# SamArgt/AudioSourceSep

Measured on AMD Instinct MI355X. Metric: Glow fwd+logdet passes/sec on 64×64×1 mel tiles (K=32,L=3), 1→8 MI355X, higher is better.
Workload: dtype f16x3

## Files before the change

### audiosourcesep_amd/csrc/glowk_co.h

```cpp
#pragma once
#include "glowk_kernels.h"

constexpr int CO_PX = 128;
constexpr int CO_PSTR = 132;

template <int KIN, int MOUT, int NF, int MODE>
struct RingC {
  static constexpr int MODE7 = net_dir<MODE>;
  using S = RingS<KIN, MOUT, NF, MODE7, 2>;
  static constexpr bool FUSE = (MODE & NET_FUSE) != 0;
  static constexpr bool SAVE = MODE7 == NET_FWD_SAVE, BWD = MODE7 == NET_BWD;
  static constexpr bool MERGE = S::NMT <= 3;
  static constexpr bool M0LAST = S::NMT % 3 == 2;
  static constexpr bool STORE = (MODE & NET_STORE) != 0;
  static constexpr int MODEX = net_dir<MODE> | (MODE & NET_STORE);
  static constexpr int NFH = S::NFH, NRB = S::NRB, NMT = S::NMT, KS = S::KS;
  static constexpr int UNITP = S::MAINP / 2;
  static constexpr int UNIT4 = S::MAIN4 / 2;
  static constexpr int PPW = UNITP / 4;
  static constexpr int NG = NFH / 2;
  static constexpr int K1PW = (S::K1P + 3) / 4;
  static constexpr int EPN = BWD ? 0 : S::EPN;
  static constexpr int MASKN = BWD ? 2 * 4 * NF * 64 : 0;
  static constexpr size_t LDS_BYTES = (size_t)3 * UNIT4 * 16 + (size_t)2 * S::K14 * 16 + (size_t)EPN * 4 + (size_t)MASKN * 2 +
                                      (FUSE ? (size_t)36 * CO_PSTR * 4 + CO_PX * 16 : 0);
  static constexpr bool FITS = (MODE7 == NET_FWD || MODE7 == NET_FWD2 || SAVE || BWD) && !(MODE & NET_HALF) && (!STORE || ((SAVE || BWD) && !FUSE)) && S::NGRP == 1 && (NMT == 2 || NMT == 3 || (NMT == 5 && !STORE && !BWD)) &&
                               (!FUSE || (MOUT == 36 && !BWD)) && KS <= 3 && NF % 4 == 0 && NFH >= 2 && NFH % 2 == 0 && UNITP % 4 == 0 && PPW == NG &&
                               2 * LDS_BYTES <= 160 * 1024 + 1;
  static constexpr int XST = STORE ? 8 : 0;
  static constexpr int z_acts(int z) { int n = 0; for (int t = z * NFH; t < (z + 1) * NFH; ++t) n += (t % NMT == 0) ? 1 : 0; return n; }
  static constexpr int z_st(int z) { return STORE ? z_acts(z) * (8 + (SAVE ? 1 : 0)) : 0; }
  __device__ static const float4* main_unit(const float4* img, int pass, int i, int half) { return S::main_chunk(img, pass, i) + (size_t)half * UNIT4; }
  __device__ static const float4* out_unit(const float4* img, int pass, int z) { return S::out_chunk(img, pass, 0) + (size_t)z * UNIT4; }
};

__device__ __forceinline__ void co_bar() {
  __builtin_amdgcn_s_waitcnt(0xC07F);
  h3_barrier();
}

template <int N>
__device__ __forceinline__ void co_end() {
  __builtin_amdgcn_s_waitcnt((N & 15) | 0x0070 | ((N >> 4) << 14));
  h3_barrier();
}
template <int N>
__device__ __forceinline__ void co_end_st(bool more) {
  if (more) co_end<N + 1>();
  else co_end<N>();
}
// ... 38 lines not shown
    acc2[o1][1] = __builtin_amdgcn_mfma_f32_16x16x32_f16(af[3], bh[1], acc2[o1][1], 0, 0, 0);
    if (MODE7 != NET_FWD2) {
      acc2[o0][0] = __builtin_amdgcn_mfma_f32_16x16x32_f16(af[0], bl[0], acc2[o0][0], 0, 0, 0);
      acc2[o0][1] = __builtin_amdgcn_mfma_f32_16x16x32_f16(af[0], bl[1], acc2[o0][1], 0, 0, 0);
      acc2[o1][0] = __builtin_amdgcn_mfma_f32_16x16x32_f16(af[2], bl[0], acc2[o1][0], 0, 0, 0);
      acc2[o1][1] = __builtin_amdgcn_mfma_f32_16x16x32_f16(af[2], bl[1], acc2[o1][1], 0, 0, 0);
    }
    acc2[o0][0] = __builtin_amdgcn_mfma_f32_16x16x32_f16(af[0], bh[0], acc2[o0][0], 0, 0, 0);
    acc2[o0][1] = __builtin_amdgcn_mfma_f32_16x16x32_f16(af[0], bh[1], acc2[o0][1], 0, 0, 0);
    acc2[o1][0] = __builtin_amdgcn_mfma_f32_16x16x32_f16(af[2], bh[0], acc2[o1][0], 0, 0, 0);
    acc2[o1][1] = __builtin_amdgcn_mfma_f32_16x16x32_f16(af[2], bh[1], acc2[o1][1], 0, 0, 0);
    __builtin_amdgcn_sched_barrier(0);
  }
}

template <int KIN, int MOUT, int NF, int MODE, int PASS, bool SOLO, int Z>
__device__ __forceinline__ void co_Z(const NetArgs& a, const H3Ctx& hc, const CoCtx& c, const float* epl, float* pl,
                                     f32x4 (&acc2)[(RingC<KIN, MOUT, NF, MODE>::NRB)][2], f32x4 (&acc3)[(RingC<KIN, MOUT, NF, MODE>::NMT)][2], h8 (&bh)[2],
                                     h8 (&bl)[2], const int (&q)[2], const bool (&qok)[2], int lane, int kq,
                                     f32x4 (&keep)[(RingC<KIN, MOUT, NF, MODE>::NMT)][2]) {
  using G = RingC<KIN, MOUT, NF, MODE>;
  constexpr int NFH = G::NFH, NMT = G::NMT, M3 = MOUT, MODE7 = G::MODE7;
  constexpr bool NEXT = !SOLO && PASS == 0;
  constexpr bool LAST = !SOLO && PASS == 1;
  if constexpr (NMT == 3) {
    if constexpr (Z == 0) stage4<G::UNITP, 70>(G::out_unit(c.img, PASS, 2), c.m1, c.w4, c.voff);
    if constexpr (Z == 1 && NEXT) stage4<G::UNITP, 71>(G::out_unit(c.img, PASS + 1, 0), c.d, c.w4, c.voff);
    if constexpr (Z == 2 && NEXT) stage4<G::UNITP, 72>(G::main_unit(c.img, PASS + 1, 0, 0), c.m0, c.w4, c.voff);
  } else if constexpr (NMT == 2) {
    if constexpr (Z == 0 && NEXT) stage4<G::UNITP, 75>(G::main_unit(c.img, PASS + 1, 0, 1), c.m1, c.w4, c.voff);
    if constexpr (Z == 1 && NEXT) stage4<G::UNITP, 76>(G::out_unit(c.img, PASS + 1, 0), c.d, c.w4, c.voff);
  } else {
    static_assert(NMT == 5, "conv3 units");
    if constexpr (Z == 0) stage4<G::UNITP, 80>(G::out_unit(c.img, PASS, 2), c.m1, c.w4, c.voff);
    if constexpr (Z == 1) stage4<G::UNITP, 81>(G::out_unit(c.img, PASS, 3), c.d, c.w4, c.voff);
    if constexpr (Z == 2) stage4<G::UNITP, 82>(G::out_unit(c.img, PASS, 4), c.m0, c.w4, c.voff);
    if constexpr (Z == 3 && NEXT) stage4<G::UNITP, 83>(G::main_unit(c.img, PASS + 1, 0, 1), c.m1, c.w4, c.voff);
    if constexpr (Z == 4 && NEXT) stage4<G::UNITP, 84>(G::out_unit(c.img, PASS + 1, 0), c.d, c.w4, c.voff);
  }
  const float4* slot = Z % 3 == 0 ? c.d : Z % 3 == 1 ? c.m0 : c.m1;
  const h8* buf = reinterpret_cast<const h8*>(slot) + lane;
  const float* pb = epl + NF * 32;
#pragma unroll
  for (int tp = 0; tp < NFH; ++tp) {
    const int t = Z * NFH + tp;
    const int fo = t / NMT, ml = t % NMT;
    if (ml == 0) {
      unsigned mask = 0, bits = 0;
      if (G::BWD) mask = hc.mkl[((size_t)(threadIdx.x >> 6) * NF + PASS * NFH + fo) * 64 + lane];
      if constexpr (G::STORE)
        bits = h3s_act_pair<MODE7, true>(acc2[2 * fo][0], acc2[2 * fo + 1][0], acc2[2 * fo][1], acc2[2 * fo + 1][1], a.sc2, mask, bh, bl,
                                         uniform_fptr(a.st2 + (size_t)(PASS * NFH + fo) * 32 * a.Q), ((unsigned)(4 * kq) * (unsigned)a.Q + (unsigned)q[0]) * 4u,
                                         (unsigned)a.Q * 4u);
// ... 16 lines not shown
#pragma unroll
        for (int r = 0; r < 4; ++r) {
          const int m = ml * 16 + 4 * kq + r;
          const float part = G::BWD ? acc3[ml][hf][r] * (a.sc3 * hc.ub[hf]) : PASS == 0 ? fmaf(acc3[ml][hf][r], a.sc3, pb[m]) : acc3[ml][hf][r] * a.sc3;
          if constexpr (NEXT && G::MERGE) { keep[ml][hf][r] = part; continue; }
          const float val = (LAST && G::MERGE) ? part + keep[ml][hf][r] : part;
          if constexpr (G::FUSE) {
            if (m < M3) pl[m * CO_PSTR + (int)(threadIdx.x >> 6) * 32 + 16 * hf + (lane & 15)] = val;
          } else {
            float* Pp = a.P + ((SOLO || !G::MERGE) ? (size_t)PASS * a.pstride : (size_t)0);
            if (m < M3 && qok[hf]) Pp[(size_t)m * a.Q + q[hf]] = val;
          }
        }
    }
  }
  constexpr bool ISSUED = NMT == 3 ? (Z == 0 || NEXT) : NMT == 2 ? (Z <= 1 && NEXT) : (Z <= 2 || NEXT);
  if constexpr (Z + 1 < NMT) {
    if constexpr (G::STORE) {
      constexpr int after = (ISSUED ? G::PPW : 0) + G::z_st(Z) + ((NMT == 3 && Z == 1) ? G::z_st(0) : 0);
      co_end<(after < 63 ? after : 63)>();
    } else if constexpr (G::SAVE) co_end<0>();
    else co_end<(ISSUED ? G::PPW : 0)>();
  } else co_bar();
}

template <int KIN, int MOUT, int NF, int MODE, int PASS, bool SOLO>
__device__ __forceinline__ void co_pass(const NetArgs& a, const H3Ctx& hc, const CoCtx& c, const float* epl, float* pl,
                                        const h8 (&xh)[(RingC<KIN, MOUT, NF, MODE>::KS)][2], const h8 (&xl)[(RingC<KIN, MOUT, NF, MODE>::KS)][2],
                                        const int (&q)[2], const bool (&qok)[2], int lane, int kq, f32x4 (&keep)[(RingC<KIN, MOUT, NF, MODE>::NMT)][2]) {
  using G = RingC<KIN, MOUT, NF, MODE>;
  using S = typename G::S;
  constexpr int NRB = G::NRB, NFH = G::NFH, MODE7 = G::MODE7;
  constexpr int f2base = PASS * NFH * 32;
  constexpr bool SECOND = !SOLO && PASS == 1;
  f32x4 acc2[NRB][2];
#pragma unroll
  for (int ob = 0; ob < NRB; ++ob)
#pragma unroll
    for (int r = 0; r < 4; ++r) {
      const float b = G::BWD ? 0.0f : epl[f2base + ob * 16 + 4 * kq + r];
      acc2[ob][0][r] = b;
      acc2[ob][1][r] = b;
    }
  const bool st = G::SAVE && PASS == 0 && hc.wok;
  constexpr int XST = PASS == 0 ? G::XST : 0;
  h8 bh[2], bl[2];
#pragma nounroll
  for (int i0 = 0; i0 < NF; i0 += 2) {
    if (i0 > 0 || (SECOND && !G::M0LAST)) stage4<G::UNITP, 73>(G::main_unit(c.img, PASS, i0, 1), c.m1, c.w4, c.voff);
// ... 5 lines not shown
    else co_end_st<G::PPW + XST>(st);
    co_Y<NFH, MODE7, 0, 1, S::K1P>(c.m0, bh, bl, acc2, lane, hc.k1img + (size_t)((i0 + 2) % NF) * S::K14, hc.k1s0, c.w4, c.voff);
    co_end_st<G::K1PW + XST>(st);
    co_Y<NFH, MODE7, 1, 2, S::K1P>(c.m1, bh, bl, acc2, lane, G::main_unit(c.img, PASS, i0 + 1, 0), c.m0, c.w4, c.voff);
    co_bar();
    stage4<G::UNITP, 74>(G::main_unit(c.img, PASS, i0 + 1, 1), c.m1, c.w4, c.voff);
    h3s_X<KIN, MOUT, NF, G::MODEX, 2, 1, PASS, G::STORE>(a, hc, i0 + 1, xh, xl, lane, bh, bl);
    co_end_st<G::PPW + XST>(st);
    co_Y<NFH, MODE7, 0, 3, S::K1P>(c.m0, bh, bl, acc2, lane, hc.k1img + (size_t)((i0 + 3) % NF) * S::K14, hc.k1s1, c.w4, c.voff);
    co_end_st<G::K1PW + XST>(st);
    co_Y<NFH, MODE7, 1, 4, S::K1P>(c.m1, bh, bl, acc2, lane, i0 + 2 < NF ? G::main_unit(c.img, PASS, i0 + 2, 0) : G::out_unit(c.img, PASS, 1), c.m0,
                                   c.w4, c.voff);
    co_bar();
  }
  f32x4 acc3[G::NMT][2];
  co_Z<KIN, MOUT, NF, MODE, PASS, SOLO, 0>(a, hc, c, epl, pl, acc2, acc3, bh, bl, q, qok, lane, kq, keep);
  co_Z<KIN, MOUT, NF, MODE, PASS, SOLO, 1>(a, hc, c, epl, pl, acc2, acc3, bh, bl, q, qok, lane, kq, keep);
  if constexpr (G::NMT >= 3) co_Z<KIN, MOUT, NF, MODE, PASS, SOLO, 2>(a, hc, c, epl, pl, acc2, acc3, bh, bl, q, qok, lane, kq, keep);
  if constexpr (G::NMT >= 4) co_Z<KIN, MOUT, NF, MODE, PASS, SOLO, 3>(a, hc, c, epl, pl, acc2, acc3, bh, bl, q, qok, lane, kq, keep);
  if constexpr (G::NMT >= 5) co_Z<KIN, MOUT, NF, MODE, PASS, SOLO, 4>(a, hc, c, epl, pl, acc2, acc3, bh, bl, q, qok, lane, kq, keep);
}

template <int KIN, int MOUT, int NF, int MODE, bool SPLIT>
__global__ __launch_bounds__(256, 2) void k_net_h3c(NetArgs a) {
  using G = RingC<KIN, MOUT, NF, MODE>;
  using S = typename G::S;
  constexpr int KS = G::KS;
  constexpr int SGN = G::BWD ? -1 : 1;
  static_assert(G::FITS, "shape");
  static_assert(!(G::FUSE && SPLIT), "the fused coupling needs both passes in one workgroup");

  const int tid = threadIdx.x;
  __shared__ __attribute__((aligned(1024))) float4 slotM0[G::UNIT4];
  __shared__ __attribute__((aligned(1024))) float4 slotM1[G::UNIT4];
  __shared__ __attribute__((aligned(1024))) float4 slotD[G::UNIT4];
  __shared__ __attribute__((aligned(1024))) float4 k1slot0[S::K14];
  __shared__ __attribute__((aligned(1024))) float4 k1slot1[S::K14];
  float* epl = nullptr;
  if constexpr (!G::BWD) { __shared__ float epl_arr[S::EPN]; epl = epl_arr; }
  unsigned short* mkl = nullptr;
  if constexpr (G::BWD) { __shared__ __attribute__((aligned(1024))) unsigned short mkl_arr[G::MASKN]; mkl = mkl_arr; }
  float* plds = nullptr;
  float4* vstash = nullptr;
  if constexpr (G::FUSE) {
    __shared__ float plds_arr[36 * CO_PSTR];
// ... 6 lines not shown
  const int kq = lane >> 4;
  const int qbase = ((int)blockIdx.x * 4 + wave) * 32;
  const int q[2] = {G::STORE ? qbase + 2 * n16 : qbase + n16, G::STORE ? qbase + 2 * n16 + 1 : qbase + 16 + n16};
  const bool qok[2] = {q[0] < a.Q, q[1] < a.Q};
  const int pass0 = SPLIT ? (int)blockIdx.y : 0;

  H3Ctx hc;
  hc.sA = hc.sB = hc.sD = nullptr; hc.k1s0 = k1slot0; hc.k1s1 = k1slot1;
  hc.k1img = a.RSp; hc.img = a.RSp; hc.mkl = mkl; hc.mk2off = 4 * NF * 64; hc.pl = plds;
  hc.wblk = (size_t)blockIdx.x * 4 + wave;
  hc.wok = (long)hc.wblk * 32 < a.Q;
  hc.w4 = wave; hc.voff = (unsigned)lane * 16u; hc.ub[0] = hc.ub[1] = 1.0f;
  CoCtx c;
  c.m0 = slotM0; c.m1 = slotM1; c.d = slotD; c.img = a.RSp; c.w4 = wave; c.voff = (unsigned)lane * 16u;

  stage4<G::UNITP, 60>(G::main_unit(c.img, pass0, 0, 0), slotM0, c.w4, c.voff);
  stage4<G::UNITP, 61>(G::main_unit(c.img, pass0, 0, 1), slotM1, c.w4, c.voff);
  stage4<G::UNITP, 62>(G::out_unit(c.img, pass0, 0), slotD, c.w4, c.voff);
  stage4<S::K1P, 63>(hc.k1img, k1slot0, c.w4, c.voff);
  stage4<S::K1P, 64>(hc.k1img + S::K14, k1slot1, c.w4, c.voff);
  if constexpr (G::BWD) {
    stage4<NF / 2, 65>(reinterpret_cast<const float4*>(a.mask1 + (size_t)blockIdx.x * 4 * NF * 64), reinterpret_cast<float4*>(mkl), c.w4, c.voff);
    stage4<NF / 2, 66>(reinterpret_cast<const float4*>(a.mask2 + (size_t)blockIdx.x * 4 * NF * 64), reinterpret_cast<float4*>(mkl + 4 * NF * 64), c.w4, c.voff);
  }

  h8 xh[KS][2], xl[KS][2];
  float xmax = 0.0f;
  {
    const int hw = a.h * a.w;
#pragma unroll
    for (int hf = 0; hf < 2; ++hf) {
      const int qq = qok[hf] ? q[hf] : 0;
      const int rem = qq % hw;
      const int i = rem / a.w, j0 = rem % a.w;
      const float* base = a.vin + (long)qq * a.in_stride + a.in_off;
      if constexpr (G::BWD) {
        float v[KS][8];
        float pm = 0.0f;
#pragma unroll
        for (int s = 0; s < KS; ++s) {
          gather8<KIN, false, SGN>(base, i, j0, a.h, a.w, a.in_stride, qok[hf], 32 * s + 8 * kq, v[s]);
          pm = range8(pm, v[s]);
        }
        pm = nan_max(pm, __shfl_xor(pm, 16, 64));
        pm = nan_max(pm, __shfl_xor(pm, 32, 64));
        xmax = nan_max(xmax, pm);
        const float fac = G::STORE ? 1.0f : pixel_norm(pm, a.bnorm, hc.ub[hf]);
#pragma unroll
        for (int s = 0; s < KS; ++s) {
#pragma unroll
          for (int j = 0; j < 8; ++j) v[s][j] *= fac;
          split8(v[s], xh[s][hf], xl[s][hf]);
        }
      } else if constexpr (S::STK) {
        xmax = gather_stacked<KIN, SGN, G::MODE7 == NET_FWD2, KS, S::KSX>(base, i, j0, a.h, a.w, a.in_stride, qok[hf], kq, xh, xl, hf, xmax);
      } else {
#pragma unroll
        for (int s = 0; s < KS; ++s) {
          float v[8];
          gather8<KIN, true, SGN>(base, i, j0, a.h, a.w, a.in_stride, qok[hf], 32 * s + 8 * kq, v);
          xmax = range8(xmax, v);
          split8(v, xh[s][hf], xl[s][hf]);
        }
      }
    }
  }
  if constexpr (G::FUSE) {
    if (tid < CO_PX) {
      const int qv = (int)blockIdx.x * CO_PX + tid;
      vstash[tid] = qv < a.Q ? *reinterpret_cast<const float4*>(a.vin + (size_t)qv * 4) : float4{0.f, 0.f, 0.f, 0.f};
    }
  }
  if constexpr (!G::BWD)
    for (int i = tid; i < S::EPN; i += 256) epl[i] = a.eph[i];
  if (((G::BWD && !G::STORE) ? !(xmax <= 3.0e38f) : !(xmax <= a.xlim)) && a.flag) *a.flag = 1;
  if (a.xmax_out) range_probe(a.xmax_out, xmax);
  asm volatile("s_waitcnt vmcnt(0)" ::: "memory");
  __syncthreads();

  f32x4 keep[G::NMT][2];
  if constexpr (SPLIT) {
    if (pass0 == 0) co_pass<KIN, MOUT, NF, MODE, 0, true>(a, hc, c, epl, plds, xh, xl, q, qok, lane, kq, keep);
    else co_pass<KIN, MOUT, NF, MODE, 1, true>(a, hc, c, epl, plds, xh, xl, q, qok, lane, kq, keep);
  } else {
    co_pass<KIN, MOUT, NF, MODE, 0, false>(a, hc, c, epl, plds, xh, xl, q, qok, lane, kq, keep);
    co_pass<KIN, MOUT, NF, MODE, 1, false>(a, hc, c, epl, plds, xh, xl, q, qok, lane, kq, keep);
  }
  if constexpr (G::FUSE) {
    __syncthreads();
    fused_couple<CO_PX, CO_PSTR>(a, plds, vstash, tid);
  }
}
```

### audiosourcesep_amd/csrc/glowk_kernels.h

```cpp
#pragma once
#include "glowk_act_scale.h"

#include <hip/hip_runtime.h>
#include <utility>
#include <stdint.h>

typedef float f32x16 __attribute__((ext_vector_type(16)));

#define GLOWK_GPTR(p) ((const __attribute__((address_space(1))) void*)(p))
#define GLOWK_LPTR(p) ((__attribute__((address_space(3))) void*)(p))

__device__ __forceinline__ int mfma_row(int r, int hh) { return (r & 3) + 8 * (r >> 2) + 4 * hh; }

struct NetArgs {
  const float* vin;
  int in_stride, in_off;
  int Q, h, w;
  const float* K1p;
  const float* ep;
  const float4* R0p;
  unsigned short* mask1;
  unsigned short* mask2;
  float* P;
  size_t pstride;
// ... 1225 lines not shown
  f32x4 acc3[G::G0N][2];
  h3s_tail<KIN, MOUT, NF, MODE, NP, P0, PASS, SOLO>(a, c, epl, acc2, acc3, bh, bl, g, q, qok, lane, kq, keep, std::make_integer_sequence<int, 2 * G::NCH>());
}

template <int KIN, int MOUT, int NF, int MODE, int NP, int PASS, int P0>
__device__ __forceinline__ void h3s_passes(const NetArgs& a, const H3Ctx& c, const float* epl, const h8 (&xh)[(RingS<KIN, MOUT, NF, MODE, NP>::KS)][2],
                                           const h8 (&xl)[(RingS<KIN, MOUT, NF, MODE, NP>::KS)][2], int g, const int (&q)[2], const bool (&qok)[2], int lane, int kq,
                                           f32x4 (&keep)[(RingS<KIN, MOUT, NF, MODE, NP>::G0N)][2]) {
  h3s_pass<KIN, MOUT, NF, MODE, NP, P0, PASS, false>(a, c, epl, xh, xl, g, q, qok, lane, kq, keep);
  if constexpr (PASS + 1 < NP) h3s_passes<KIN, MOUT, NF, MODE, NP, PASS + 1, (RingS<KIN, MOUT, NF, MODE, NP>::NCH + 1 + P0) & 1>(a, c, epl, xh, xl, g, q, qok, lane, kq, keep);
}

__device__ __forceinline__ bool fz_not_finite(float v) { return !(fabsf(v) <= 3.0e38f); }

template <int PXW = 256, int PSTR = FUSE_PSTR>
__device__ __forceinline__ void fused_couple(const NetArgs& a, const float* pl, const float4* vst, int tid) {
  const int wave = tid >> 6, lane = tid & 63;
  const int px = wave * 32 + (lane & 31), k = lane >> 5;
  const int q = (int)blockIdx.x * PXW + px;
  const bool qok = q < a.Q;
  const int w = a.w, hw = a.h * a.w, nrows = PXW / w;
  const int pp = (qok ? q : 0) % hw;
  const int i = pp / w, j = pp % w, r = px / w;
  float ols = 0.0f, ot = 0.0f;
  bool missing = false;
#pragma unroll
  for (int tap = 0; tap < 9; ++tap) {
    const int dy = tap / 3 - 1, dx = tap % 3 - 1;
    const int ii = i + dy, jj = j + dx;
    if (ii < 0 || ii >= a.h || jj < 0 || jj >= w) continue;
    const int rr = r + dy;
    if (rr < 0 || rr >= nrows) { missing = true; continue; }
    const int spx = px + dy * w + dx;
    ols += pl[(tap * 4 + k) * PSTR + spx];
// ... 15 lines not shown
    bool bad = fz_not_finite(ols) | fz_not_finite(ot) | fz_not_finite(yk);
    if (bad && a.flag) *a.flag = 1;
    float z0, z1;
    if (a.fz_A) {
      z0 = a.fz_b[2 * k]; z1 = a.fz_b[2 * k + 1];
#pragma unroll
      for (int ci = 0; ci < 4; ++ci) {
        z0 = fmaf(y[ci], a.fz_A[ci * 4 + 2 * k], z0);
        z1 = fmaf(y[ci], a.fz_A[ci * 4 + 2 * k + 1], z1);
      }
    } else {
      z0 = y[2 * k]; z1 = y[2 * k + 1];
    }
    *reinterpret_cast<float2*>(a.fz_out + (size_t)q * a.fz_out_stride + a.fz_out_off + 2 * k) = float2{z0, z1};
  } else if (qok) {
    float* e = a.fz_edge + (((size_t)blockIdx.x * 4 + (r == 0 ? 0 : 1)) * FUSE_EW + j) * 4;
    e[k] = ols;
    e[2 + k] = ot;
  }
  for (int te = tid; te < 2 * w * 4; te += 2 * PXW) {
    const int which = te / (4 * w), jt = (te / 4) % w, ch = te & 3;
    float hsum = 0.0f;
#pragma unroll
    for (int dx = -1; dx <= 1; ++dx) {
      const int js = jt + dx;
      if (js < 0 || js >= w) continue;
      const int tap = (which ? 0 : 6) + dx + 1;
      hsum += pl[(tap * 4 + ch) * PSTR + (which ? (nrows - 1) * w : 0) + js];
    }
    a.fz_edge[(((size_t)blockIdx.x * 4 + 2 + which) * FUSE_EW + jt) * 4 + ch] = hsum;
  }
  if (a.fz_ldpart) {
    double d = (double)lsum;
#pragma unroll
    for (int o = 32; o > 0; o >>= 1) d += __shfl_down(d, o, 64);
    if (lane == 0) a.fz_ldpart[(size_t)blockIdx.x * (PXW / 32) + wave] = d;
  }
}

template <int KIN, int MOUT, int NF, int MODE, int NP, bool SPLIT>
__global__ __launch_bounds__(512, 2) void k_net_h3s(NetArgs a) {
  using G = RingS<KIN, MOUT, NF, MODE, NP>;
  constexpr int KS = G::KS;
  constexpr int SGN = (net_dir<MODE> == NET_BWD) ? -1 : 1;
  static_assert(G::FITS, "shape");

  __shared__ float4 slotA[G::MAIN4];
  __shared__ float4 slotB[G::MAIN4];
  __shared__ float4 slotD[G::MAIN4];
  __shared__ float4 k1slot0[G::K14];
  __shared__ float4 k1slot1[G::K14];
// ... 97 lines not shown
  f32x4 keep[G::G0N][2];
  if (g) h3_barrier();
  if constexpr (SPLIT) {
    if (solo_pass == 0) h3s_pass<KIN, MOUT, NF, MODE, NP, 0, 0, true>(a, c, epl, xh, xl, g, q, qok, lane, kq, keep);
    else if (solo_pass == 1) h3s_pass<KIN, MOUT, NF, MODE, NP, 0, 1, true>(a, c, epl, xh, xl, g, q, qok, lane, kq, keep);
    else if constexpr (NP > 2) {
      if (solo_pass == 2) h3s_pass<KIN, MOUT, NF, MODE, NP, 0, 2, true>(a, c, epl, xh, xl, g, q, qok, lane, kq, keep);
      else h3s_pass<KIN, MOUT, NF, MODE, NP, 0, 3, true>(a, c, epl, xh, xl, g, q, qok, lane, kq, keep);
    }
  } else {
    h3s_passes<KIN, MOUT, NF, MODE, NP, 0, 0>(a, c, epl, xh, xl, g, q, qok, lane, kq, keep);
  }
  if (!g) h3_barrier();
  if constexpr (G::FUSE) {
    __syncthreads();
    fused_couple(a, plds, vstash, tid);
  }
}
```

### audiosourcesep_amd/csrc/glowk_launch.h

```cpp
#pragma once
#include "glowk_kernels.h"
#include "glowk_co.h"
#include "glowk_q.h"

#include <cstdlib>
#include <string>

#define GLOWK_NET_SHAPES(X) X(2, 16) X(4, 16) X(8, 16) X(16, 16) X(2, 12) X(4, 12) X(8, 12) X(16, 12) \
                            X(2, 8) X(4, 8) X(8, 8) X(16, 8) X(2, 4) X(4, 4) X(8, 4) X(16, 4)

enum NetArith { NET_EXACT, NET_SPLIT3, NET_SPLIT2 };
struct NetCall { int dir; NetArith arith; bool store = false; };

enum NetFamily { FAM_F32, FAM_H3, FAM_H3S, FAM_H3S_HALF, FAM_FUSED, FAM_CO, FAM_Q, FAM_COUNT };

struct NetLaunch {
  int np = 0;
  int family = FAM_F32;
  bool co = false;
  bool q = false;
  int fused_px = 0;
  bool failed = false;
  explicit operator bool() const { return np > 0 || fused_px > 0; }
};
// ... 53 lines not shown
  return {};
}

template <class Kernel>
inline bool co_two_per_cu(Kernel kernel) {
  static int blocks = -1;
  if (blocks < 0) {
    int n = 0;
    if (hipOccupancyMaxActiveBlocksPerMultiprocessor(&n, kernel, 256, 0) != hipSuccess) { (void)hipGetLastError(); n = 0; }
    blocks = n;
  }
  return blocks >= 2;
}

template <int KIN, int MOUT, int NF, int MODE>
NetLaunch launch_h3s(const NetArgs& a, hipStream_t s, bool dry) {
  static_assert(!(MODE & NET_STORE), "no storing launches here: the co-resident branch does not check Q % 128 (launch_co_train does)");
  constexpr bool F2 = RingS<KIN, MOUT, NF, MODE, 2>::FITS, F4 = RingS<KIN, MOUT, NF, MODE, 4>::FITS;
  const int wgs = (a.Q + 255) / 256, cus = num_cus();
  if constexpr (F4) {
    if (a.max_np >= 4 && (4 * wgs <= cus || !F2)) {
      const bool split = 4 * wgs <= cus;
      if (!dry) {
        if (split) hipLaunchKernelGGL((k_net_h3s<KIN, MOUT, NF, MODE, 4, true>), dim3(wgs, 4), dim3(512), 0, s, a);
        else hipLaunchKernelGGL((k_net_h3s<KIN, MOUT, NF, MODE, 4, false>), dim3(wgs), dim3(512), 0, s, a);
      }
      return {4, FAM_H3S};
    }
  }
  if constexpr (F2) {
    const bool split = 2 * wgs <= cus;
    if constexpr (RingC<KIN, MOUT, NF, MODE>::FITS) {
      const int wgc = (a.Q + CO_PX - 1) / CO_PX;
      const bool co_ok = a.co && !env().co_off;
      if (co_ok && wgc > cus) {
        if constexpr (RingC<KIN, MOUT, NF, MODE | NET_FUSE>::FITS) {
          if (a.fuse && co_two_per_cu(k_net_h3c<KIN, MOUT, NF, MODE | NET_FUSE, false>)) {
            if (!dry) hipLaunchKernelGGL((k_net_h3c<KIN, MOUT, NF, MODE | NET_FUSE, false>), dim3(wgc), dim3(256), 0, s, a);
            return {0, FAM_FUSED, true, false, CO_PX};
          }
        }
        if (!a.fuse && co_two_per_cu(k_net_h3c<KIN, MOUT, NF, MODE, false>)) {
          if (!dry) hipLaunchKernelGGL((k_net_h3c<KIN, MOUT, NF, MODE, false>), dim3(wgc), dim3(256), 0, s, a);
          return {RingC<KIN, MOUT, NF, MODE>::MERGE ? 1 : 2, FAM_H3S, true};
        }
      }
      if (co_ok && split && wgc <= cus && a.max_np >= 2 && co_two_per_cu(k_net_h3c<KIN, MOUT, NF, MODE, true>)) {
        if (!dry) hipLaunchKernelGGL((k_net_h3c<KIN, MOUT, NF, MODE, true>), dim3(wgc, 2), dim3(256), 0, s, a);
        return {2, FAM_H3S, true};
      }
    }
    if constexpr ((MODE == NET_FWD || MODE == NET_FWD2 || MODE == NET_FWD_SAVE) && MOUT == 36) {
      if constexpr (RingS<KIN, MOUT, NF, MODE | NET_FUSE, 2>::FITS && RingS<KIN, MOUT, NF, MODE | NET_FUSE, 2>::MERGE) {
        if (a.fuse && !split) {
          if (!dry) hipLaunchKernelGGL((k_net_h3s<KIN, MOUT, NF, MODE | NET_FUSE, 2, false>), dim3(wgs), dim3(512), 0, s, a);
          return {0, FAM_FUSED, false, false, 256};
        }
      }
// ... 170 lines not shown
```

Before: 15960.

## Make co-resident forward net kernel persistent with cross-block weight and input prefetch

Forward co-resident net kernels with stacked input now run as persistent workgroups. The grid is capped at two per CU and each workgroup loops over pixel blocks. During the second pass the next block's first weight units are prefetched into LDS, and the next block's input gather is issued before the fused coupling epilogue, so the prologue of each new block overlaps the tail of the previous one. This is meant to hide per-workgroup startup costs: staging weights, gathering inputs, loading epilogue parameters, and launching many waves. In exchange it adds loop control, more registers to hold in-flight inputs, and conditional wait counts, and it threads an explicit block index through fused_couple.

```diff
diff --git a/audiosourcesep_amd/csrc/glowk_co.h b/audiosourcesep_amd/csrc/glowk_co.h
--- a/audiosourcesep_amd/csrc/glowk_co.h
+++ b/audiosourcesep_amd/csrc/glowk_co.h
@@ -34,6 +34,9 @@
   __device__ static const float4* out_unit(const float4* img, int pass, int z) { return S::out_chunk(img, pass, 0) + (size_t)z * UNIT4; }
 };
 
+template <int KIN, int MOUT, int NF, int MODE, bool SPLIT>
+constexpr bool co_persistent = !SPLIT && (net_dir<MODE> == NET_FWD || net_dir<MODE> == NET_FWD2) && !(MODE & NET_STORE) && RingC<KIN, MOUT, NF, MODE>::S::STK;
+
 __device__ __forceinline__ void co_bar() {
   __builtin_amdgcn_s_waitcnt(0xC07F);
   h3_barrier();
@@ -102,29 +105,33 @@
   }
 }
 
-template <int KIN, int MOUT, int NF, int MODE, int PASS, bool SOLO, int Z>
+template <int KIN, int MOUT, int NF, int MODE, int PASS, bool SOLO, int Z, bool PERS = false>
 __device__ __forceinline__ void co_Z(const NetArgs& a, const H3Ctx& hc, const CoCtx& c, const float* epl, float* pl,
                                      f32x4 (&acc2)[(RingC<KIN, MOUT, NF, MODE>::NRB)][2], f32x4 (&acc3)[(RingC<KIN, MOUT, NF, MODE>::NMT)][2], h8 (&bh)[2],
                                      h8 (&bl)[2], const int (&q)[2], const bool (&qok)[2], int lane, int kq,
-                                     f32x4 (&keep)[(RingC<KIN, MOUT, NF, MODE>::NMT)][2]) {
+                                     f32x4 (&keep)[(RingC<KIN, MOUT, NF, MODE>::NMT)][2], bool more = false) {
   using G = RingC<KIN, MOUT, NF, MODE>;
   constexpr int NFH = G::NFH, NMT = G::NMT, M3 = MOUT, MODE7 = G::MODE7;
+  constexpr bool NEXTB = PERS && !SOLO && PASS == 1;
   constexpr bool NEXT = !SOLO && PASS == 0;
+  constexpr bool NEXTD = NEXT || NEXTB;
   constexpr bool LAST = !SOLO && PASS == 1;
+  constexpr int NPASS = NEXTB ? 0 : PASS + 1;
+  const bool nx = !NEXTB || more;
   if constexpr (NMT == 3) {
     if constexpr (Z == 0) stage4<G::UNITP, 70>(G::out_unit(c.img, PASS, 2), c.m1, c.w4, c.voff);
-    if constexpr (Z == 1 && NEXT) stage4<G::UNITP, 71>(G::out_unit(c.img, PASS + 1, 0), c.d, c.w4, c.voff);
-    if constexpr (Z == 2 && NEXT) stage4<G::UNITP, 72>(G::main_unit(c.img, PASS + 1, 0, 0), c.m0, c.w4, c.voff);
+    if constexpr (Z == 1 && NEXTD) { if (nx) stage4<G::UNITP, 71>(G::out_unit(c.img, NPASS, 0), c.d, c.w4, c.voff); }
+    if constexpr (Z == 2 && NEXTD) { if (nx) stage4<G::UNITP, 72>(G::main_unit(c.img, NPASS, 0, 0), c.m0, c.w4, c.voff); }
   } else if constexpr (NMT == 2) {
-    if constexpr (Z == 0 && NEXT) stage4<G::UNITP, 75>(G::main_unit(c.img, PASS + 1, 0, 1), c.m1, c.w4, c.voff);
-    if constexpr (Z == 1 && NEXT) stage4<G::UNITP, 76>(G::out_unit(c.img, PASS + 1, 0), c.d, c.w4, c.voff);
+    if constexpr (Z == 0 && NEXTD) { if (nx) stage4<G::UNITP, 75>(G::main_unit(c.img, NPASS, 0, 1), c.m1, c.w4, c.voff); }
+    if constexpr (Z == 1 && NEXTD) { if (nx) stage4<G::UNITP, 76>(G::out_unit(c.img, NPASS, 0), c.d, c.w4, c.voff); }
   } else {
     static_assert(NMT == 5, "conv3 units");
     if constexpr (Z == 0) stage4<G::UNITP, 80>(G::out_unit(c.img, PASS, 2), c.m1, c.w4, c.voff);
     if constexpr (Z == 1) stage4<G::UNITP, 81>(G::out_unit(c.img, PASS, 3), c.d, c.w4, c.voff);
     if constexpr (Z == 2) stage4<G::UNITP, 82>(G::out_unit(c.img, PASS, 4), c.m0, c.w4, c.voff);
-    if constexpr (Z == 3 && NEXT) stage4<G::UNITP, 83>(G::main_unit(c.img, PASS + 1, 0, 1), c.m1, c.w4, c.voff);
-    if constexpr (Z == 4 && NEXT) stage4<G::UNITP, 84>(G::out_unit(c.img, PASS + 1, 0), c.d, c.w4, c.voff);
+    if constexpr (Z == 3 && NEXTD) { if (nx) stage4<G::UNITP, 83>(G::main_unit(c.img, NPASS, 0, 1), c.m1, c.w4, c.voff); }
+    if constexpr (Z == 4 && NEXTD) { if (nx) stage4<G::UNITP, 84>(G::out_unit(c.img, NPASS, 0), c.d, c.w4, c.voff); }
   }
   const float4* slot = Z % 3 == 0 ? c.d : Z % 3 == 1 ? c.m0 : c.m1;
   const h8* buf = reinterpret_cast<const h8*>(slot) + lane;
@@ -171,25 +178,29 @@
         }
     }
   }
-  constexpr bool ISSUED = NMT == 3 ? (Z == 0 || NEXT) : NMT == 2 ? (Z <= 1 && NEXT) : (Z <= 2 || NEXT);
+  constexpr bool ISSUED = NMT == 3 ? (Z == 0 || NEXTD) : NMT == 2 ? (Z <= 1 && NEXTD) : (Z <= 2 || NEXTD);
   if constexpr (Z + 1 < NMT) {
     if constexpr (G::STORE) {
       constexpr int after = (ISSUED ? G::PPW : 0) + G::z_st(Z) + ((NMT == 3 && Z == 1) ? G::z_st(0) : 0);
       co_end<(after < 63 ? after : 63)>();
     } else if constexpr (G::SAVE) co_end<0>();
-    else co_end<(ISSUED ? G::PPW : 0)>();
+    else if constexpr (NEXTB && (NMT == 3 ? Z >= 1 : NMT == 2 ? true : Z >= 3)) {
+      if (more) co_end<G::PPW>();
+      else co_end<0>();
+    } else co_end<(ISSUED ? G::PPW : 0)>();
   } else co_bar();
 }
 
-template <int KIN, int MOUT, int NF, int MODE, int PASS, bool SOLO>
+template <int KIN, int MOUT, int NF, int MODE, int PASS, bool SOLO, bool PERS = false>
 __device__ __forceinline__ void co_pass(const NetArgs& a, const H3Ctx& hc, const CoCtx& c, const float* epl, float* pl,
                                         const h8 (&xh)[(RingC<KIN, MOUT, NF, MODE>::KS)][2], const h8 (&xl)[(RingC<KIN, MOUT, NF, MODE>::KS)][2],
-                                        const int (&q)[2], const bool (&qok)[2], int lane, int kq, f32x4 (&keep)[(RingC<KIN, MOUT, NF, MODE>::NMT)][2]) {
+                                        const int (&q)[2], const bool (&qok)[2], int lane, int kq, f32x4 (&keep)[(RingC<KIN, MOUT, NF, MODE>::NMT)][2],
+                                        bool more = false) {
   using G = RingC<KIN, MOUT, NF, MODE>;
   using S = typename G::S;
   constexpr int NRB = G::NRB, NFH = G::NFH, MODE7 = G::MODE7;
   constexpr int f2base = PASS * NFH * 32;
-  constexpr bool SECOND = !SOLO && PASS == 1;
+  constexpr bool SECOND = (!SOLO && PASS == 1) || PERS;
   f32x4 acc2[NRB][2];
 #pragma unroll
   for (int ob = 0; ob < NRB; ++ob)
@@ -225,11 +236,108 @@
     co_bar();
   }
   f32x4 acc3[G::NMT][2];
-  co_Z<KIN, MOUT, NF, MODE, PASS, SOLO, 0>(a, hc, c, epl, pl, acc2, acc3, bh, bl, q, qok, lane, kq, keep);
-  co_Z<KIN, MOUT, NF, MODE, PASS, SOLO, 1>(a, hc, c, epl, pl, acc2, acc3, bh, bl, q, qok, lane, kq, keep);
-  if constexpr (G::NMT >= 3) co_Z<KIN, MOUT, NF, MODE, PASS, SOLO, 2>(a, hc, c, epl, pl, acc2, acc3, bh, bl, q, qok, lane, kq, keep);
-  if constexpr (G::NMT >= 4) co_Z<KIN, MOUT, NF, MODE, PASS, SOLO, 3>(a, hc, c, epl, pl, acc2, acc3, bh, bl, q, qok, lane, kq, keep);
-  if constexpr (G::NMT >= 5) co_Z<KIN, MOUT, NF, MODE, PASS, SOLO, 4>(a, hc, c, epl, pl, acc2, acc3, bh, bl, q, qok, lane, kq, keep);
+  co_Z<KIN, MOUT, NF, MODE, PASS, SOLO, 0, PERS>(a, hc, c, epl, pl, acc2, acc3, bh, bl, q, qok, lane, kq, keep, more);
+  co_Z<KIN, MOUT, NF, MODE, PASS, SOLO, 1, PERS>(a, hc, c, epl, pl, acc2, acc3, bh, bl, q, qok, lane, kq, keep, more);
+  if constexpr (G::NMT >= 3) co_Z<KIN, MOUT, NF, MODE, PASS, SOLO, 2, PERS>(a, hc, c, epl, pl, acc2, acc3, bh, bl, q, qok, lane, kq, keep, more);
+  if constexpr (G::NMT >= 4) co_Z<KIN, MOUT, NF, MODE, PASS, SOLO, 3, PERS>(a, hc, c, epl, pl, acc2, acc3, bh, bl, q, qok, lane, kq, keep, more);
+  if constexpr (G::NMT >= 5) co_Z<KIN, MOUT, NF, MODE, PASS, SOLO, 4, PERS>(a, hc, c, epl, pl, acc2, acc3, bh, bl, q, qok, lane, kq, keep, more);
+}
+
+template <int KSX>
+struct CoIn {
+  float x[2][KSX][8];
+  int i[2], j0[2];
+  float4 v4;
+};
+
+template <int KIN, int KSX, bool FUSE>
+__device__ __forceinline__ void co_in_issue(const NetArgs& a, int blk, int wave, int n16, int kq, int tid, CoIn<KSX>& in) {
+  constexpr int K1 = 9 * KIN;
+  constexpr int G = KIN < 8 ? KIN : 8;
+  static_assert(G == 2 || G == 4, "channel group");
+  const int hw = a.h * a.w;
+  const int qbase = (blk * 4 + wave) * 32;
+#pragma unroll
+  for (int hf = 0; hf < 2; ++hf) {
+    const int qp = qbase + 16 * hf + n16;
+    const bool qok = qp < a.Q;
+    const int qq = qok ? qp : 0;
+    const int rem = qq % hw;
+    const int i = rem / a.w, j0 = rem % a.w;
+    in.i[hf] = i; in.j0[hf] = j0;
+    const float* base = a.vin + (long)qq * a.in_stride + a.in_off;
+#pragma unroll
+    for (int sx = 0; sx < KSX; ++sx)
+#pragma unroll
+      for (int t = 0; t < 8 / G; ++t) {
+        const int p = 32 * sx + 8 * kq + t * G;
+        const int seg = p / K1, k = p - seg * K1;
+        const int tap = k / KIN, cin = k % KIN;
+        const int dy = tap / 3 - 1, dx = tap % 3 - 1;
+        const int ii = i + dy, jj = j0 + dx;
+        const bool ok = qok && seg < 3 && ii >= 0 && ii < a.h && jj >= 0 && jj < a.w;
+        const float* ptr = base + (ok ? (dy * a.w + dx) * a.in_stride + cin : 0);
+        if constexpr (G == 4) {
+          const float4 v = *reinterpret_cast<const float4*>(ptr);
+          in.x[hf][sx][t * 4 + 0] = v.x; in.x[hf][sx][t * 4 + 1] = v.y; in.x[hf][sx][t * 4 + 2] = v.z; in.x[hf][sx][t * 4 + 3] = v.w;
+        } else {
+          const float2 v = *reinterpret_cast<const float2*>(ptr);
+          in.x[hf][sx][t * 2 + 0] = v.x; in.x[hf][sx][t * 2 + 1] = v.y;
+        }
+      }
+  }
+  if constexpr (FUSE) {
+    const int qv = blk * CO_PX + (tid & (CO_PX - 1));
+    in.v4 = *reinterpret_cast<const float4*>(a.vin + (size_t)(qv < a.Q ? qv : 0) * 4);
+  }
+}
+
+template <int KIN, bool TWO, int KS, int KSX, bool FUSE>
+__device__ __forceinline__ float co_in_split(const NetArgs& a, int blk, int wave, int n16, int kq, int tid, const CoIn<KSX>& in, h8 (&xh)[KS][2],
+                                             h8 (&xl)[KS][2], float4* vstash, float xmax) {
+  constexpr int K1 = 9 * KIN;
+  constexpr int G = KIN < 8 ? KIN : 8;
+  const int qbase = (blk * 4 + wave) * 32;
+#pragma unroll
+  for (int hf = 0; hf < 2; ++hf) {
+    const bool qok = qbase + 16 * hf + n16 < a.Q;
+    const int i = in.i[hf], j0 = in.j0[hf];
+#pragma unroll
+    for (int sx = 0; sx < 2 * KS; ++sx) {
+      h8& f = (sx & 1) ? xl[sx >> 1][hf] : xh[sx >> 1][hf];
+      if (sx >= KSX) {
+#pragma unroll
+        for (int j = 0; j < 8; ++j) f[j] = (_Float16)0.0f;
+        continue;
+      }
+#pragma unroll
+      for (int t = 0; t < 8 / G; ++t) {
+        const int p = 32 * sx + 8 * kq + t * G;
+        const int seg = p / K1, k = p - seg * K1;
+        const int tap = k / KIN;
+        const int ii = i + tap / 3 - 1, jj = j0 + tap % 3 - 1;
+        const bool ok = qok && seg < 3 && ii >= 0 && ii < a.h && jj >= 0 && jj < a.w;
+        int okv = ok ? -1 : 0, cbv = p == 3 * K1 ? __float_as_int(GLOWK_ACT_SCALE) : 0;
+        asm volatile("" : "+v"(okv), "+v"(cbv));
+#pragma unroll
+        for (int e = 0; e < G; e += 2) {
+          const int cbe = e == 0 ? cbv : 0;
+          const float x0 = in.x[hf][sx][t * G + e], x1 = in.x[hf][sx][t * G + e + 1];
+          const f32x2 v = {__int_as_float((__float_as_int(x0 * GLOWK_ACT_SCALE) & okv) | cbe), __int_as_float((__float_as_int(x1 * GLOWK_ACT_SCALE) & okv) | cbe)};
+          xmax = nan_max(nan_max(xmax, __builtin_fabsf(v.x)), __builtin_fabsf(v.y));
+          const h2v hi = __builtin_convertvector(v, h2v);
+          const h2v lo = __builtin_convertvector(v - __builtin_convertvector(hi, f32x2), h2v);
+          const h2v z = {(_Float16)0.0f, (_Float16)0.0f};
+          const h2v sel = seg == 1 ? (TWO ? z : lo) : hi;
+          f[t * G + e] = sel[0]; f[t * G + e + 1] = sel[1];
+        }
+      }
+    }
+  }
+  if constexpr (FUSE) {
+    if (tid < CO_PX) vstash[tid] = blk * CO_PX + tid < a.Q ? in.v4 : float4{0.f, 0.f, 0.f, 0.f};
+  }
+  return xmax;
 }
 
 template <int KIN, int MOUT, int NF, int MODE, bool SPLIT>
@@ -240,6 +348,7 @@
   constexpr int SGN = G::BWD ? -1 : 1;
   static_assert(G::FITS, "shape");
   static_assert(!(G::FUSE && SPLIT), "the fused coupling needs both passes in one workgroup");
+  constexpr bool PERS = co_persistent<KIN, MOUT, NF, MODE, SPLIT>;
 
   const int tid = threadIdx.x;
   __shared__ __attribute__((aligned(1024))) float4 slotM0[G::UNIT4];
@@ -276,80 +385,128 @@
   CoCtx c;
   c.m0 = slotM0; c.m1 = slotM1; c.d = slotD; c.img = a.RSp; c.w4 = wave; c.voff = (unsigned)lane * 16u;
 
-  stage4<G::UNITP, 60>(G::main_unit(c.img, pass0, 0, 0), slotM0, c.w4, c.voff);
-  stage4<G::UNITP, 61>(G::main_unit(c.img, pass0, 0, 1), slotM1, c.w4, c.voff);
-  stage4<G::UNITP, 62>(G::out_unit(c.img, pass0, 0), slotD, c.w4, c.voff);
-  stage4<S::K1P, 63>(hc.k1img, k1slot0, c.w4, c.voff);
-  stage4<S::K1P, 64>(hc.k1img + S::K14, k1slot1, c.w4, c.voff);
-  if constexpr (G::BWD) {
-    stage4<NF / 2, 65>(reinterpret_cast<const float4*>(a.mask1 + (size_t)blockIdx.x * 4 * NF * 64), reinterpret_cast<float4*>(mkl), c.w4, c.voff);
-    stage4<NF / 2, 66>(reinterpret_cast<const float4*>(a.mask2 + (size_t)blockIdx.x * 4 * NF * 64), reinterpret_cast<float4*>(mkl + 4 * NF * 64), c.w4, c.voff);
-  }
-
-  h8 xh[KS][2], xl[KS][2];
-  float xmax = 0.0f;
-  {
-    const int hw = a.h * a.w;
-#pragma unroll
-    for (int hf = 0; hf < 2; ++hf) {
-      const int qq = qok[hf] ? q[hf] : 0;
-      const int rem = qq % hw;
-      const int i = rem / a.w, j0 = rem % a.w;
-      const float* base = a.vin + (long)qq * a.in_stride + a.in_off;
-      if constexpr (G::BWD) {
-        float v[KS][8];
-        float pm = 0.0f;
-#pragma unroll
-        for (int s = 0; s < KS; ++s) {
-          gather8<KIN, false, SGN>(base, i, j0, a.h, a.w, a.in_stride, qok[hf], 32 * s + 8 * kq, v[s]);
-          pm = range8(pm, v[s]);
+  if constexpr (PERS) {
+    if constexpr (G::M0LAST) stage4<G::UNITP, 61>(G::main_unit(c.img, 0, 0, 1), slotM1, c.w4, c.voff);
+    else stage4<G::UNITP, 60>(G::main_unit(c.img, 0, 0, 0), slotM0, c.w4, c.voff);
+    stage4<G::UNITP, 62>(G::out_unit(c.img, 0, 0), slotD, c.w4, c.voff);
+    stage4<S::K1P, 63>(hc.k1img, k1slot0, c.w4, c.voff);
+    stage4<S::K1P, 64>(hc.k1img + S::K14, k1slot1, c.w4, c.voff);
+    const int nblk = (a.Q + CO_PX - 1) / CO_PX, grid = (int)gridDim.x;
+    int blk = (int)blockIdx.x;
+    CoIn<S::KSX> in0;
+    co_in_issue<KIN, S::KSX, G::FUSE>(a, blk, wave, n16, kq, tid, in0);
+    for (int i = tid; i < S::EPN; i += 256) epl[i] = a.eph[i];
+    h8 xh[KS][2], xl[KS][2];
+    float xmax = 0.0f;
+    xmax = co_in_split<KIN, G::MODE7 == NET_FWD2, KS, S::KSX, G::FUSE>(a, blk, wave, n16, kq, tid, in0, xh, xl, vstash, xmax);
+    asm volatile("s_waitcnt vmcnt(0)" ::: "memory");
+    __syncthreads();
+    f32x4 keep[G::NMT][2];
+    for (;;) {
+      int tb = tid;
+      asm volatile("" : "+v"(tb));
+      const int ln = tb & 63, kb = ln >> 4, nb = ln & 15;
+      c.voff = hc.voff = (unsigned)ln * 16u;
+      const int qb = (blk * 4 + wave) * 32;
+      const int q[2] = {qb + nb, qb + 16 + nb};
+      const bool qok[2] = {q[0] < a.Q, q[1] < a.Q};
+      const int nxt = blk + grid;
+      const bool more = __builtin_amdgcn_readfirstlane(nxt < nblk ? 1 : 0) != 0;
+      co_pass<KIN, MOUT, NF, MODE, 0, false, true>(a, hc, c, epl, plds, xh, xl, q, qok, ln, kb, keep);
+      co_pass<KIN, MOUT, NF, MODE, 1, false, true>(a, hc, c, epl, plds, xh, xl, q, qok, ln, kb, keep, more);
+      int tt = tid;
+      asm volatile("" : "+v"(tt));
+      const int kt = (tt & 63) >> 4, nt = tt & 15;
+      CoIn<S::KSX> in;
+      co_in_issue<KIN, S::KSX, G::FUSE>(a, more ? nxt : blk, wave, nt, kt, tt, in);
+      if constexpr (G::FUSE) {
+        co_bar();
+        fused_couple<CO_PX, CO_PSTR>(a, plds, vstash, tt, blk);
+      }
+      if (!more) break;
+      if constexpr (G::FUSE) co_bar();
+      blk = nxt;
+      xmax = co_in_split<KIN, G::MODE7 == NET_FWD2, KS, S::KSX, G::FUSE>(a, blk, wave, nt, kt, tt, in, xh, xl, vstash, xmax);
+    }
+    if (!(xmax <= a.xlim) && a.flag) *a.flag = 1;
+    if (a.xmax_out) range_probe(a.xmax_out, xmax);
+    asm volatile("s_waitcnt vmcnt(0)" ::: "memory");
+  } else {
+    stage4<G::UNITP, 60>(G::main_unit(c.img, pass0, 0, 0), slotM0, c.w4, c.voff);
+    stage4<G::UNITP, 61>(G::main_unit(c.img, pass0, 0, 1), slotM1, c.w4, c.voff);
+    stage4<G::UNITP, 62>(G::out_unit(c.img, pass0, 0), slotD, c.w4, c.voff);
+    stage4<S::K1P, 63>(hc.k1img, k1slot0, c.w4, c.voff);
+    stage4<S::K1P, 64>(hc.k1img + S::K14, k1slot1, c.w4, c.voff);
+    if constexpr (G::BWD) {
+      stage4<NF / 2, 65>(reinterpret_cast<const float4*>(a.mask1 + (size_t)blockIdx.x * 4 * NF * 64), reinterpret_cast<float4*>(mkl), c.w4, c.voff);
+      stage4<NF / 2, 66>(reinterpret_cast<const float4*>(a.mask2 + (size_t)blockIdx.x * 4 * NF * 64), reinterpret_cast<float4*>(mkl + 4 * NF * 64), c.w4, c.voff);
+    }
+
+    h8 xh[KS][2], xl[KS][2];
+    float xmax = 0.0f;
+    {
+      const int hw = a.h * a.w;
+  #pragma unroll
+      for (int hf = 0; hf < 2; ++hf) {
+        const int qq = qok[hf] ? q[hf] : 0;
+        const int rem = qq % hw;
+        const int i = rem / a.w, j0 = rem % a.w;
+        const float* base = a.vin + (long)qq * a.in_stride + a.in_off;
+        if constexpr (G::BWD) {
+          float v[KS][8];
+          float pm = 0.0f;
+  #pragma unroll
+          for (int s = 0; s < KS; ++s) {
+            gather8<KIN, false, SGN>(base, i, j0, a.h, a.w, a.in_stride, qok[hf], 32 * s + 8 * kq, v[s]);
+            pm = range8(pm, v[s]);
+          }
+          pm = nan_max(pm, __shfl_xor(pm, 16, 64));
+          pm = nan_max(pm, __shfl_xor(pm, 32, 64));
+          xmax = nan_max(xmax, pm);
+          const float fac = G::STORE ? 1.0f : pixel_norm(pm, a.bnorm, hc.ub[hf]);
+  #pragma unroll
+          for (int s = 0; s < KS; ++s) {
+  #pragma unroll
+            for (int j = 0; j < 8; ++j) v[s][j] *= fac;
+            split8(v[s], xh[s][hf], xl[s][hf]);
+          }
+        } else if constexpr (S::STK) {
+          xmax = gather_stacked<KIN, SGN, G::MODE7 == NET_FWD2, KS, S::KSX>(base, i, j0, a.h, a.w, a.in_stride, qok[hf], kq, xh, xl, hf, xmax);
+        } else {
+  #pragma unroll
+          for (int s = 0; s < KS; ++s) {
+            float v[8];
+            gather8<KIN, true, SGN>(base, i, j0, a.h, a.w, a.in_stride, qok[hf], 32 * s + 8 * kq, v);
+            xmax = range8(xmax, v);
+            split8(v, xh[s][hf], xl[s][hf]);
+          }
         }
-        pm = nan_max(pm, __shfl_xor(pm, 16, 64));
-        pm = nan_max(pm, __shfl_xor(pm, 32, 64));
-        xmax = nan_max(xmax, pm);
-        const float fac = G::STORE ? 1.0f : pixel_norm(pm, a.bnorm, hc.ub[hf]);
-#pragma unroll
-        for (int s = 0; s < KS; ++s) {
-#pragma unroll
-          for (int j = 0; j < 8; ++j) v[s][j] *= fac;
-          split8(v[s], xh[s][hf], xl[s][hf]);
-        }
-      } else if constexpr (S::STK) {
-        xmax = gather_stacked<KIN, SGN, G::MODE7 == NET_FWD2, KS, S::KSX>(base, i, j0, a.h, a.w, a.in_stride, qok[hf], kq, xh, xl, hf, xmax);
-      } else {
-#pragma unroll
-        for (int s = 0; s < KS; ++s) {
-          float v[8];
-          gather8<KIN, true, SGN>(base, i, j0, a.h, a.w, a.in_stride, qok[hf], 32 * s + 8 * kq, v);
-          xmax = range8(xmax, v);
-          split8(v, xh[s][hf], xl[s][hf]);
-        }
-      }
-    }
-  }
-  if constexpr (G::FUSE) {
-    if (tid < CO_PX) {
-      const int qv = (int)blockIdx.x * CO_PX + tid;
-      vstash[tid] = qv < a.Q ? *reinterpret_cast<const float4*>(a.vin + (size_t)qv * 4) : float4{0.f, 0.f, 0.f, 0.f};
-    }
-  }
-  if constexpr (!G::BWD)
-    for (int i = tid; i < S::EPN; i += 256) epl[i] = a.eph[i];
-  if (((G::BWD && !G::STORE) ? !(xmax <= 3.0e38f) : !(xmax <= a.xlim)) && a.flag) *a.flag = 1;
-  if (a.xmax_out) range_probe(a.xmax_out, xmax);
-  asm volatile("s_waitcnt vmcnt(0)" ::: "memory");
-  __syncthreads();
-
-  f32x4 keep[G::NMT][2];
-  if constexpr (SPLIT) {
-    if (pass0 == 0) co_pass<KIN, MOUT, NF, MODE, 0, true>(a, hc, c, epl, plds, xh, xl, q, qok, lane, kq, keep);
-    else co_pass<KIN, MOUT, NF, MODE, 1, true>(a, hc, c, epl, plds, xh, xl, q, qok, lane, kq, keep);
-  } else {
-    co_pass<KIN, MOUT, NF, MODE, 0, false>(a, hc, c, epl, plds, xh, xl, q, qok, lane, kq, keep);
-    co_pass<KIN, MOUT, NF, MODE, 1, false>(a, hc, c, epl, plds, xh, xl, q, qok, lane, kq, keep);
-  }
-  if constexpr (G::FUSE) {
+      }
+    }
+    if constexpr (G::FUSE) {
+      if (tid < CO_PX) {
+        const int qv = (int)blockIdx.x * CO_PX + tid;
+        vstash[tid] = qv < a.Q ? *reinterpret_cast<const float4*>(a.vin + (size_t)qv * 4) : float4{0.f, 0.f, 0.f, 0.f};
+      }
+    }
+    if constexpr (!G::BWD)
+      for (int i = tid; i < S::EPN; i += 256) epl[i] = a.eph[i];
+    if (((G::BWD && !G::STORE) ? !(xmax <= 3.0e38f) : !(xmax <= a.xlim)) && a.flag) *a.flag = 1;
+    if (a.xmax_out) range_probe(a.xmax_out, xmax);
+    asm volatile("s_waitcnt vmcnt(0)" ::: "memory");
     __syncthreads();
-    fused_couple<CO_PX, CO_PSTR>(a, plds, vstash, tid);
-  }
-}
+
+    f32x4 keep[G::NMT][2];
+    if constexpr (SPLIT) {
+      if (pass0 == 0) co_pass<KIN, MOUT, NF, MODE, 0, true>(a, hc, c, epl, plds, xh, xl, q, qok, lane, kq, keep);
+      else co_pass<KIN, MOUT, NF, MODE, 1, true>(a, hc, c, epl, plds, xh, xl, q, qok, lane, kq, keep);
+    } else {
+      co_pass<KIN, MOUT, NF, MODE, 0, false>(a, hc, c, epl, plds, xh, xl, q, qok, lane, kq, keep);
+      co_pass<KIN, MOUT, NF, MODE, 1, false>(a, hc, c, epl, plds, xh, xl, q, qok, lane, kq, keep);
+    }
+    if constexpr (G::FUSE) {
+      __syncthreads();
+      fused_couple<CO_PX, CO_PSTR>(a, plds, vstash, tid, (int)blockIdx.x);
+    }
+  }
+}
diff --git a/audiosourcesep_amd/csrc/glowk_kernels.h b/audiosourcesep_amd/csrc/glowk_kernels.h
--- a/audiosourcesep_amd/csrc/glowk_kernels.h
+++ b/audiosourcesep_amd/csrc/glowk_kernels.h
@@ -1263,10 +1263,10 @@
 __device__ __forceinline__ bool fz_not_finite(float v) { return !(fabsf(v) <= 3.0e38f); }
 
 template <int PXW = 256, int PSTR = FUSE_PSTR>
-__device__ __forceinline__ void fused_couple(const NetArgs& a, const float* pl, const float4* vst, int tid) {
+__device__ __forceinline__ void fused_couple(const NetArgs& a, const float* pl, const float4* vst, int tid, int blk) {
   const int wave = tid >> 6, lane = tid & 63;
   const int px = wave * 32 + (lane & 31), k = lane >> 5;
-  const int q = (int)blockIdx.x * PXW + px;
+  const int q = blk * PXW + px;
   const bool qok = q < a.Q;
   const int w = a.w, hw = a.h * a.w, nrows = PXW / w;
   const int pp = (qok ? q : 0) % hw;
@@ -1312,7 +1312,7 @@
     }
     *reinterpret_cast<float2*>(a.fz_out + (size_t)q * a.fz_out_stride + a.fz_out_off + 2 * k) = float2{z0, z1};
   } else if (qok) {
-    float* e = a.fz_edge + (((size_t)blockIdx.x * 4 + (r == 0 ? 0 : 1)) * FUSE_EW + j) * 4;
+    float* e = a.fz_edge + (((size_t)blk * 4 + (r == 0 ? 0 : 1)) * FUSE_EW + j) * 4;
     e[k] = ols;
     e[2 + k] = ot;
   }
@@ -1326,13 +1326,13 @@
       const int tap = (which ? 0 : 6) + dx + 1;
       hsum += pl[(tap * 4 + ch) * PSTR + (which ? (nrows - 1) * w : 0) + js];
     }
-    a.fz_edge[(((size_t)blockIdx.x * 4 + 2 + which) * FUSE_EW + jt) * 4 + ch] = hsum;
+    a.fz_edge[(((size_t)blk * 4 + 2 + which) * FUSE_EW + jt) * 4 + ch] = hsum;
   }
   if (a.fz_ldpart) {
     double d = (double)lsum;
 #pragma unroll
     for (int o = 32; o > 0; o >>= 1) d += __shfl_down(d, o, 64);
-    if (lane == 0) a.fz_ldpart[(size_t)blockIdx.x * (PXW / 32) + wave] = d;
+    if (lane == 0) a.fz_ldpart[(size_t)blk * (PXW / 32) + wave] = d;
   }
 }
 
@@ -1460,6 +1460,6 @@
   if (!g) h3_barrier();
   if constexpr (G::FUSE) {
     __syncthreads();
-    fused_couple(a, plds, vstash, tid);
-  }
-}
+    fused_couple(a, plds, vstash, tid, (int)blockIdx.x);
+  }
+}
diff --git a/audiosourcesep_amd/csrc/glowk_launch.h b/audiosourcesep_amd/csrc/glowk_launch.h
--- a/audiosourcesep_amd/csrc/glowk_launch.h
+++ b/audiosourcesep_amd/csrc/glowk_launch.h
@@ -3,6 +3,7 @@
 #include "glowk_co.h"
 #include "glowk_q.h"
 
+#include <algorithm>
 #include <cstdlib>
 #include <string>
 
@@ -91,6 +92,11 @@
 }
 
 template <int KIN, int MOUT, int NF, int MODE>
+inline int co_grid(int wgc, int cus) {
+  return co_persistent<KIN, MOUT, NF, MODE, false> ? std::min(wgc, 2 * cus) : wgc;
+}
+
+template <int KIN, int MOUT, int NF, int MODE>
 NetLaunch launch_h3s(const NetArgs& a, hipStream_t s, bool dry) {
   static_assert(!(MODE & NET_STORE), "no storing launches here: the co-resident branch does not check Q % 128 (launch_co_train does)");
   constexpr bool F2 = RingS<KIN, MOUT, NF, MODE, 2>::FITS, F4 = RingS<KIN, MOUT, NF, MODE, 4>::FITS;
@@ -113,12 +119,12 @@
       if (co_ok && wgc > cus) {
         if constexpr (RingC<KIN, MOUT, NF, MODE | NET_FUSE>::FITS) {
           if (a.fuse && co_two_per_cu(k_net_h3c<KIN, MOUT, NF, MODE | NET_FUSE, false>)) {
-            if (!dry) hipLaunchKernelGGL((k_net_h3c<KIN, MOUT, NF, MODE | NET_FUSE, false>), dim3(wgc), dim3(256), 0, s, a);
+            if (!dry) hipLaunchKernelGGL((k_net_h3c<KIN, MOUT, NF, MODE | NET_FUSE, false>), dim3(co_grid<KIN, MOUT, NF, MODE | NET_FUSE>(wgc, cus)), dim3(256), 0, s, a);
             return {0, FAM_FUSED, true, false, CO_PX};
           }
         }
         if (!a.fuse && co_two_per_cu(k_net_h3c<KIN, MOUT, NF, MODE, false>)) {
-          if (!dry) hipLaunchKernelGGL((k_net_h3c<KIN, MOUT, NF, MODE, false>), dim3(wgc), dim3(256), 0, s, a);
+          if (!dry) hipLaunchKernelGGL((k_net_h3c<KIN, MOUT, NF, MODE, false>), dim3(co_grid<KIN, MOUT, NF, MODE>(wgc, cus)), dim3(256), 0, s, a);
           return {RingC<KIN, MOUT, NF, MODE>::MERGE ? 1 : 2, FAM_H3S, true};
         }
       }
```

New measurement: 15560. 0.975x the previous value.
